# AO33/HiC_Genome_Assembler

Measured on AMD Instinct MI355X. Metric: Part1+Part2 wall-clock (s) and bins/s on N x N contact map, higher is better.
Workload: dtype f64

## Files before the change

hic_genome_assembler_amd/csrc/api.hip:

```cpp
#include <hip/hip_runtime.h>

#include <algorithm>
#include <cmath>
#include <cstdarg>
#include <climits>
#include <cstdio>
#include <cstdlib>
#include <cstring>
#include <numeric>
#include <string>
#include <type_traits>
#include <unordered_map>
#include <functional>
#include <chrono>
#include <vector>

#include "../../include/hicmi.h"
#include "hicmi_internal.h"
#include "devbuf.h"
#include "hyper.h"

using namespace hicmi;

static thread_local std::string g_err;
// ... 2792 lines not shown
        launch_p2_total_perm(c->dM2, c->ld2, c->d_pos2sel, (int)c->n_arr, c->d_T, c->d_scores, c->stream);
    }
    HIPCHK(hipGetLastError());
    HIPCHK(hipMemcpyAsync(c->pin_down, c->d_scores, sizeof(double), hipMemcpyDeviceToHost, c->stream));
    return HICMI_OK;
}
}

int hicmi_p2_arrangement_total(hicmi_ctx* c, double* total_out)
{
    if (!c || !total_out) return fail(HICMI_EINVAL, "bad arguments");
    int rc = arrangement_total_enqueue(c);
    if (rc) return rc;
    HIPCHK(sync_stream(c));
    memcpy(total_out, c->pin_down, sizeof(double));
    return HICMI_OK;
}

int hicmi_p2_arrangement_score(hicmi_ctx* c, double total, double* score_out)
{
    if (!c || !score_out) return fail(HICMI_EINVAL, "bad arguments");
    if (c->n_arr < 1) return fail(HICMI_EINVAL, "hicmi_p2_set_arrangement has not run");
    if (c->n_arr < 2) { *score_out = 0.0; return HICMI_OK; }
    HIPCHK(hipSetDevice(c->device));
    const int NB = kBaseSlabs;
    int rc = ensure(c->d_scores, NB);
    if (rc) return rc;
    {
        Timed t(c, F_P2_SCORE, 4.0 * (double)c->n_arr * (double)(c->n_arr - 1));
        launch_p2_base_partial(c->dM2, c->ld2, c->d_pos2sel, (int)c->n_arr, c->d_H, (int)c->n_arr, NB, c->d_scores, c->stream);
    }
    HIPCHK(hipGetLastError());
    double part[NB];
    rc = download(c, part, c->d_scores, sizeof(double) * NB);
    if (rc) return rc;
    double sum = 0.0;
    for (int b = 0; b < NB; b++) sum += part[b];
    *score_out = sum / total;
    return HICMI_OK;
}

int hicmi_p2_score_insertions(hicmi_ctx* c, int32_t new_id, double total, double* scores_out)
{
    if (!c || !scores_out) return fail(HICMI_EINVAL, "bad arguments");
    if (c->n_scaf < 1) return fail(HICMI_EINVAL, "hicmi_p2_layout has not run");
    if (new_id < 0 || new_id >= c->n_scaf) return fail(HICMI_EINVAL, "new scaffold out of range");
    const int64_t S = (int64_t)c->h_arr_id.size();
    if (c->n_arr < 1 || S < 1) return fail(HICMI_EINVAL, "hicmi_p2_set_arrangement has not run");
    for (int64_t j = 0; j < S; j++) if (c->h_arr_id[(size_t)j] == new_id) return fail(HICMI_EINVAL, "scaffold is already in the arrangement");
    const int new_len = c->h_scaf_len[(size_t)new_id];
    if (int rc = check_candidate_bins(c->n_arr + new_len)) return rc;
    HIPCHK(hipSetDevice(c->device));
    const int NB = kBaseSlabs;
    const int64_t n_out = NB + S + 2 * (S + 1);
    int rc = ensure(c->d_scores, n_out);
    if (rc) return rc;
    {
        const double nn = (double)c->n_arr;
        Timed t(c, F_P2_INSERT, 8.0 * (0.5 * nn * (nn - 1.0) + nn * nn + 2.0 * (double)(S + 1) * (double)new_len * nn));
        launch_p2_insert_delta(c->dM2, c->ld2, c->d_pos2sel, (int)c->n_arr, c->d_arr_packed + S, (int)S,
                               c->h_scaf_start[(size_t)new_id], new_len, c->d_H, NB, c->d_scores, c->stream);
    }
    HIPCHK(hipGetLastError());
    std::vector<double> host((size_t)n_out);
    rc = download(c, host.data(), c->d_scores, sizeof(double) * (size_t)n_out);
    if (rc) return rc;
    double base = 0.0;
    for (int b = 0; b < NB; b++) base += host[(size_t)b];
    double straddle = 0.0;
    for (int64_t g = 0; g <= S; g++) {
        if (g > 0) straddle += host[(size_t)(NB + g - 1)];
        for (int r = 0; r < 2; r++)
            scores_out[2 * g + r] = (base - straddle + host[(size_t)(NB + S + 2 * g + r)]) / total;
    }
    return HICMI_OK;
}

int hicmi_p2_window_tables(hicmi_ctx* c, int64_t k, const int8_t* orders, int64_t n_orders, const uint8_t* orients,
                           int64_t n_orients)
{
    if (!c || !orders || !orients || k < 1 || k > 8 || n_orders < 1 || n_orients < 1) return fail(HICMI_EINVAL, "bad arguments");
    for (int64_t i = 0; i < n_orders * k; i++) if (orders[i] < 0 || orders[i] >= k) return fail(HICMI_EINVAL, "order table entry out of range");
    HIPCHK(hipSetDevice(c->device));
    int rc = ensure(c->d_orders, n_orders * k);
    if (!rc) rc = ensure(c->d_orients, n_orients * k);
    if (rc) return rc;
    rc = upload(c, c->d_orders, orders, (size_t)(n_orders * k));
    if (rc) return rc;
    rc = upload(c, c->d_orients, orients, (size_t)(n_orients * k));
    if (rc) return rc;
    c->tab_k = (int)k; c->n_orders = n_orders; c->n_orients = n_orients;
    c->h_orders.assign(orders, orders + n_orders * k);
    c->h_orients.assign(orients, orients + n_orients * k);
    return HICMI_OK;
}

namespace {
int64_t window_c0(const hicmi_ctx* c, int64_t first, int64_t k)
{
    for (int64_t r = 0; r < c->n_orients; r++) {
        bool same = true;
        for (int64_t j = 0; j < k; j++) same = same && ((c->h_orients[(size_t)(r * k + j)] != 0) == (c->h_arr_rev[(size_t)(first + j)] != 0));
        if (same) return r;
    }
    return -1;
}

struct BatchCost { int64_t g_total = 0; int max_m = 0; double g_bytes = 0.0, d_bytes = 0.0, g_flops = 0.0; };

int fill_batch(hicmi_ctx* c, int64_t first0, int64_t count, int64_t k, std::vector<WindowBatchEntry>& wb, BatchCost& bc)
{
    const int64_t S = (int64_t)c->h_arr_id.size();
    if (c->n_arr < 1 || S < 1) return fail(HICMI_EINVAL, "hicmi_p2_set_arrangement has not run");
    if (k != c->tab_k) return fail(HICMI_EINVAL, "hicmi_p2_window_tables has not been called for k = %lld", (long long)k);
    if (first0 < 0 || count < 1 || first0 + count - 1 + k > S) return fail(HICMI_EINVAL, "window out of range");
    const int64_t n_cand = c->n_orders * c->n_orients;
    wb.assign((size_t)count, WindowBatchEntry{});
    int64_t g_total = 0; int max_m = 0; double g_bytes = 0.0, d_bytes = 0.0, g_flops = 0.0;
    for (int64_t wdx = 0; wdx < count; wdx++) {
        const int64_t first = first0 + wdx;
        WindowBatchEntry& e = wb[(size_t)wdx];
        memset(&e, 0, sizeof(e));
        const int p0 = c->h_arr_pos[(size_t)first], p1 = c->h_arr_pos[(size_t)(first + k)];
        e.p0 = p0; e.m = p1 - p0; e.g_off = g_total;
        for (int64_t j = 0; j < k; j++) {
            const int32_t sc = c->h_arr_id[(size_t)(first + j)];
// ... 451 lines not shown
    return HICMI_OK;
}


namespace {
void apply_insertion(int32_t* ids, uint8_t* rev, int64_t& S, int64_t gap, int32_t new_id, int32_t r)
{
    for (int64_t j = S; j > gap; j--) { ids[j] = ids[j - 1]; rev[j] = rev[j - 1]; }
    ids[gap] = new_id; rev[gap] = (uint8_t)(r ? 1 : 0);
    S++;
}

struct InsJob {
    hicmi_ctx* c; int32_t* ids; uint8_t* rev; int64_t S; const int32_t* new_ids; int64_t n_new;
    int64_t t = 0; double best = 0.0; bool device_ok = true;
};

int queue_insertions(hicmi_ctx* lead, const std::vector<InsJob*>& jobs)
{
    const int nj = (int)jobs.size();
    if (nj == 0) return HICMI_OK;
    const int NB = kBaseSlabs;
    static const int max_c = getenv("HICMI_P2_INS_MAXC") ? atoi(getenv("HICMI_P2_INS_MAXC")) : INS_MAXC;
    int64_t steps_max = 0;
    std::vector<size_t> blob_off((size_t)nj);
    size_t blob_bytes = 0;
    for (int j = 0; j < nj; j++) {
        InsJob& job = *jobs[(size_t)j];
        hicmi_ctx* c = job.c;
        int rc = hicmi_p2_set_arrangement(c, job.ids, job.rev, job.S);
        if (rc) return rc;
        if (c != lead) HIPCHK(sync_stream(c));
        const int64_t n_steps = job.n_new - job.t;
        int64_t n_max = c->n_arr;
        for (int64_t t = 0; t < n_steps; t++) n_max += c->h_scaf_len[(size_t)job.new_ids[job.t + t]];
        rc = check_candidate_bins(n_max);
        if (rc) return rc;
        const int64_t S_max = job.S + n_steps;
        rc = ensure(c->d_arr_packed2, 3 * std::max<int64_t>(S_max, c->n_scaf) + 2);
        if (!rc) rc = ensure(c->d_pos2sel2, c->n2);
        if (!rc) rc = ensure(c->d_ins_T, (1 + 2 * (int64_t)INS_MAXC) * n_max);
        if (!rc) rc = ensure(c->d_ins_partial, NB + n_max + 2 * (S_max + 1));
        if (rc) return rc;
        steps_max = std::max(steps_max, n_steps);
        blob_off[(size_t)j] = blob_bytes;
        blob_bytes += (sizeof(InsState) + sizeof(InsLog) * (size_t)n_steps + 15) & ~(size_t)15;
    }
    HIPCHK(hipSetDevice(lead->device));
    int rc = ensure(lead->d_ins_blob, (int64_t)blob_bytes);
    if (!rc) rc = ensure(lead->d_ins_steps, steps_max * nj);
    if (rc) return rc;
    std::vector<InsStep> table((size_t)(steps_max * nj));
    std::vector<int> max_n_used((size_t)steps_max, 0), max_S((size_t)steps_max, 0), max_n_arr((size_t)steps_max, 0);
    double algo = 0.0;
    for (int j = 0; j < nj; j++) {
        InsJob& job = *jobs[(size_t)j];
        hicmi_ctx* c = job.c;
        const int64_t n_steps = job.n_new - job.t;
        int64_t n_max = c->n_arr;
        for (int64_t t = 0; t < n_steps; t++) n_max += c->h_scaf_len[(size_t)job.new_ids[job.t + t]];
        InsState* st = reinterpret_cast<InsState*>(lead->d_ins_blob + blob_off[(size_t)j]);
        InsLog* log = reinterpret_cast<InsLog*>(lead->d_ins_blob + blob_off[(size_t)j] + sizeof(InsState));
        int32_t* packed[2] = {c->d_arr_packed, c->d_arr_packed2};
        int32_t* pos2sel[2] = {c->d_pos2sel, c->d_pos2sel2};
        int64_t n_arr = c->n_arr;
        for (int64_t t = 0; t < steps_max; t++) {
            InsStep& d = table[(size_t)(t * nj + j)];
            memset(&d, 0, sizeof(d));
            d.st = st;
            if (t >= n_steps) continue;
            const int cur = (int)(t & 1), nxt = cur ^ 1;
            const int32_t nid = job.new_ids[job.t + t];
            const int L = c->h_scaf_len[(size_t)nid];
            d.M2 = c->dM2; d.H = c->d_H; d.ld2 = c->ld2;
            d.pos_cur = pos2sel[cur]; d.pos_nxt = pos2sel[nxt]; d.packed_cur = packed[cur]; d.packed_nxt = packed[nxt];
            d.T_total = c->d_ins_T; d.T_cand = c->d_ins_T + n_max; d.work = c->d_ins_T + (1 + (int64_t)INS_MAXC) * n_max;
            d.partial = c->d_ins_partial; d.log = log + t;
            d.n_arr = (int32_t)n_arr; d.S = (int32_t)(job.S + t); d.L = L; d.new_start = c->h_scaf_start[(size_t)nid];
            d.new_id = nid; d.active = 1; d.step = (int32_t)t; d.last = t == n_steps - 1;
            max_n_used[(size_t)t] = std::max(max_n_used[(size_t)t], (int)(n_arr + L));
            max_S[(size_t)t] = std::max(max_S[(size_t)t], d.S);
            max_n_arr[(size_t)t] = std::max(max_n_arr[(size_t)t], (int)n_arr);
            const double nn = (double)n_arr, Ld = (double)L, sd = (double)d.S;
            algo += 8.0 * (0.5 * nn * (nn - 1.0) + nn * nn + 2.0 * (sd + 1.0) * Ld * nn) + 4.0 * (nn + Ld) * (nn + Ld);
            n_arr += L;
        }
    }
    rc = upload(lead, lead->d_ins_steps, table.data(), sizeof(InsStep) * table.size());
    if (rc) return rc;
    {
        Timed timed(lead, F_P2_INSERT, algo);
        launch_insb_reset(lead->d_ins_steps, nj, lead->stream);
        for (int64_t t = 0; t < steps_max; t++) {
            const InsStep* st_t = lead->d_ins_steps + t * nj;
            const int nu = max_n_used[(size_t)t];
            launch_insb_fast(st_t, nj, max_S[(size_t)t], max_n_arr[(size_t)t], NB, lead->stream);
            launch_insb_shortlist(st_t, nj, max_S[(size_t)t], max_n_arr[(size_t)t], NB, kNearTop, max_c, lead->stream);
            launch_insb_diag_cand(st_t, nj, nu, lead->stream);
            launch_insb_cost(st_t, nj, nu, lead->stream);
            launch_insb_apply(st_t, nj, nu, lead->stream);
        }
    }
    HIPCHK(hipGetLastError());
    std::vector<unsigned char> blob(blob_bytes);
    rc = download(lead, blob.data(), lead->d_ins_blob, blob_bytes);
    if (rc) return rc;
    if (getenv("HICMI_PART2_PROFILE")) {
        int64_t hist[5] = {0, 0, 0, 0, 0}, all_direct = 0;
        for (int64_t t = 0; t < steps_max; t++) {
            int mx = -1, ran = 0;
            for (int j = 0; j < nj; j++) {
                if (t >= jobs[(size_t)j]->n_new - jobs[(size_t)j]->t) continue;
                const InsState* hs = reinterpret_cast<const InsState*>(blob.data() + blob_off[(size_t)j]);
                if (hs->fail >= 0 && t >= hs->fail) continue;
                const InsLog* hl = reinterpret_cast<const InsLog*>(blob.data() + blob_off[(size_t)j] + sizeof(InsState));
                const int ns = hl[t].n_short;
                hist[ns < 0 ? 0 : (ns > 3 ? 4 : ns + 1)]++;
                mx = std::max(mx, ns);
                ran++;
            }
            if (ran && mx < 0) all_direct++;
        }
        fprintf(stderr, "[hicmi] insertion short lists: direct %lld, literal with 0:%lld 1:%lld 2:%lld 3+:%lld candidates; "
                        "lock steps without any literal pass: %lld of %lld\n",
                (long long)hist[0], (long long)hist[1], (long long)hist[2], (long long)hist[3], (long long)hist[4],
                (long long)all_direct, (long long)steps_max);
    }
    for (int j = 0; j < nj; j++) {
        InsJob& job = *jobs[(size_t)j];
        const int64_t n_steps = job.n_new - job.t;
        const InsState* hst = reinterpret_cast<const InsState*>(blob.data() + blob_off[(size_t)j]);
        const InsLog* hlog = reinterpret_cast<const InsLog*>(blob.data() + blob_off[(size_t)j] + sizeof(InsState));
        const int64_t done = hst->fail >= 0 ? std::min<int64_t>(hst->fail, n_steps) : n_steps;
        for (int64_t t = 0; t < done; t++) {
            if (hlog[t].gap < 0 || hlog[t].gap > job.S) return fail(HICMI_ESTATE, "insertion log out of range");
            apply_insertion(job.ids, job.rev, job.S, hlog[t].gap, job.new_ids[job.t + t], hlog[t].rev);
            job.best = hlog[t].best;
        }
        job.t += done;
        hicmi_ctx* c = job.c;
        c->n_arr = 0; c->h_arr_id.clear(); c->h_arr_rev.clear(); c->h_arr_pos.clear(); c->h_pos2sel.clear();
    }
    return HICMI_OK;
}

int check_insert_job(const InsJob& job, int64_t S0)
{
    hicmi_ctx* c = job.c;
    if (!c || !job.ids || !job.rev || !job.new_ids || S0 < 1 || job.n_new < 1) return fail(HICMI_EINVAL, "bad arguments");
// ... 1278 lines not shown
```

hic_genome_assembler_amd/csrc/hicmi_internal.h:

```cpp
#pragma once
#include <hip/hip_runtime.h>
#include <stdint.h>

#include <atomic>
#include <functional>

#include "liftmap.h"
#include "span.h"
#include "ends.h"
#include "anchor.h"
#include "pairs.h"
#include "seats.h"
#include "links.h"
#include "split.h"

namespace hicmi {

inline void ensure_dynamic_lds(const void* func, std::atomic<int>& have, size_t bytes)
{
    if ((int)bytes > have.load(std::memory_order_relaxed)) {
        (void)hipFuncSetAttribute(func, hipFuncAttributeMaxDynamicSharedMemorySize, (int)bytes);
        have.store((int)bytes, std::memory_order_relaxed);
    }
}
// ... 159 lines not shown
    }
}
#endif

int  sort_padded_size(int n);
int  sort_workgroups(int n);
size_t sort_scratch_bytes(int n);
struct SortExtras {
    const int32_t* row_list = nullptr; int n_list = 0;
    uint8_t* tie_flag = nullptr; unsigned* tie_count = nullptr; unsigned tie_limit = 0;
    uint16_t* tie_bits = nullptr; int64_t ld_bits = 0;
    int max_workgroups = 0;
    int avoid_xcc = -1; unsigned* row_counter = nullptr;
};
static constexpr int GETREG_XCC_ID = 20 | (0 << 6) | (3 << 11);
int nnchain_local_xcc(const NNChainOptions& o, int n);
void launch_sort_rows(const double* C, int64_t ldc, const int32_t* order, const int32_t* inv, const double* np_sum,
                      const double* seq_sum, int n, void* scratch, uint16_t* R, int64_t ldr, int row_first, int row_stride,
                      hipStream_t s, const SortExtras& x = SortExtras());
void launch_rank_rows_tied(const uint16_t* R_storage, const uint16_t* tie_bits, int64_t ld_bits, const int32_t* order,
                           const int32_t* inv, int n, const int32_t* row_list, int n_list, uint16_t* rank, int64_t ldr,
                           hipStream_t s, int32_t* done = nullptr);
void launch_rank_relabel(const uint16_t* rank_storage, uint16_t* rank, int64_t ldr, int n, const int32_t* order, int row_first,
                         int row_stride, hipStream_t s);
size_t sort_radix_scratch_bytes(int n);
void launch_rank_rows_radix(const double* C, int64_t ldc, const int32_t* order, const int32_t* inv, const double* np_sum,
                            const double* seq_sum, int n, void* scratch, uint16_t* rank, int64_t ldr, int row_first,
                            int row_stride, hipStream_t s);
void launch_rank_invert(const uint16_t* R, uint16_t* rank, int64_t ldr, int n, int row_first, int row_stride, hipStream_t s,
                        const int32_t* row_list = nullptr, int n_list = 0);
void launch_similarity_row(const double* C, int64_t ldc, const int32_t* order, const double* np_sum,
                           const double* seq_sum, int n, int row, double* out, hipStream_t s);

void launch_p2_select(const double* C, int64_t ldc, const int32_t* sel, int n, double* M2, int64_t ld2, hipStream_t s);
void launch_p2_total(const double* M2, int64_t ld2, int n, double* T, double* total, hipStream_t s);
void launch_p2_score_exact(const double* M2, int64_t ld2, const int32_t* perms, int n_cand, int n_used, double total,
                           double* T, double* work, double* scores, hipStream_t s);
void launch_p2_score(const double* M2, int64_t ld2, const int32_t* perms, int n_cand, int n_used, const double* H,
                     double inv_total_unused, double total, double* scores, hipStream_t s);

void launch_p2_total_perm(const double* M2, int64_t ld2, const int32_t* d_perm, int n, double* T, double* total,
                          hipStream_t s);

struct WindowDesc {
    int32_t start[8];
    int32_t len[8];
    int32_t off[8];
    uint8_t rev[8];
};
void launch_arr_materialize(const int32_t* packed, int S, const int32_t* scaf_start, const int32_t* scaf_len, int n_arr,
                            int32_t* pos2sel, hipStream_t s);
void launch_p2_base_partial(const double* M2, int64_t ld2, const int32_t* pos2sel, int n_arr, const double* H, int n_tot,
                            int n_blocks, double* out, hipStream_t s);
void launch_p2_insert_delta(const double* M2, int64_t ld2, const int32_t* pos2sel, int n_arr, const int32_t* arr_pos,
                            int S, int new_start, int L, const double* H, int n_base_blocks, double* out, hipStream_t s);
struct WindowBatchEntry {
    WindowDesc w;
    int32_t p0, m;
    int64_t g_off;
    int32_t c0, pad;
};
void launch_p2_window_batch_G(const double* M2, int64_t ld2, const int32_t* pos2sel, int n, const WindowBatchEntry* wb, int n_win,
                              int max_m, const double* H, double* G_all, hipStream_t s);
void launch_p2_window_batch_delta(const double* M2, int64_t ld2, const int32_t* pos2sel, int n, int k,
                                  const WindowBatchEntry* wb, int n_win, int max_m, const int8_t* orders, const uint8_t* orients,
                                  int n_ord, int n_ori, const double* H, const double* G_all, double* delta_all, hipStream_t s);


int64_t window_table_doubles(int k);
void launch_p2_window_tables(const double* M2, int64_t ld2, const int32_t* pos2sel, int n, int k,
                             const WindowBatchEntry* wb, const WindowBatchEntry* h_wb, int n_win, int max_m, const double* H,
                             double* tables, hipStream_t s);
void launch_p2_window_candidates(int k, int n_win, const int8_t* orders, const uint8_t* orients, int n_ord, int n_ori,
                                 const double* tables, double* delta_all, hipStream_t s);
struct NearEntry { int32_t cand, pad; double fast; };
int window_near_blocks(int n_ord);
void launch_p2_window_near(const double* M2, int64_t ld2, const int32_t* pos2sel, int n, int k,
                           const WindowBatchEntry* wb, const WindowBatchEntry* h_wb, int n_win, int max_m, const int8_t* orders,
                           const uint8_t* orients, int n_ord, int n_ori, const double* H, double* tables, int whole, double total,
                           double cur_fast, double floor, double near_top, double* part, int32_t* count, NearEntry* near, int cap,
                           hipStream_t s);

__device__ __forceinline__ double wave_sum_s(double v)
{
#pragma unroll
    for (int off = 32; off >= 1; off >>= 1) v += __shfl_xor(v, off, 64);
    return v;
}

__device__ __forceinline__ double block_sum_256(double v, double* s_w)
{
    v = wave_sum_s(v);
    if ((threadIdx.x & 63) == 0) s_w[threadIdx.x >> 6] = v;
    __syncthreads();
    return (s_w[0] + s_w[1]) + (s_w[2] + s_w[3]);
}

__device__ __forceinline__ void base_partial_body(const double* __restrict__ M2, int64_t ld2, const int32_t* p, int n_arr,
                                                  const double* __restrict__ H, int n_tot, int blk, int n_blk,
                                                  double* __restrict__ out)
{
    __shared__ double s_w[4];
    const int lane = threadIdx.x & 63, wave = threadIdx.x >> 6;
    const double hn = H[n_tot - 1];
    double acc = 0.0;
    for (int a = blk * 4 + wave; a < n_arr - 1; a += n_blk * 4) {
        const double* __restrict__ row = M2 + (int64_t)p[a] * ld2;
#pragma unroll 4
// ... 12 lines not shown
    double mx = -__builtin_inf();
    int at = 0x7fffffff;
    for (int i = tid; i < n_cand; i += 256) {
        const double v = scores[i];
        if (counts(i) && isfinite(v) && v > mx) { mx = v; at = i; }
    }
    s_val[tid] = mx; s_idx[tid] = at;
    if (tid == 0) s_cnt = 0;
    __syncthreads();
    for (int w = 128; w >= 1; w >>= 1) {
        if (tid < w) {
            const double o = s_val[tid + w];
            const int oi = s_idx[tid + w];
            if (o > s_val[tid] || (o == s_val[tid] && oi < s_idx[tid])) { s_val[tid] = o; s_idx[tid] = oi; }
        }
        __syncthreads();
    }
    const double top = s_val[0];
    const int first = s_idx[0];
    if (first == 0x7fffffff) {
        if (tid == 0) { best[0] = -1; best[1] = 0; }
        return;
    }
    const double thr = top - fabs(top) * near_top;
    int near = 0;
    for (int i = tid; i < n_cand; i += 256) {
        const double v = scores[i];
        near += counts(i) && isfinite(v) && v >= thr;
    }
    if (near) atomicAdd(&s_cnt, near);
    __syncthreads();
    if (tid == 0) { best[0] = first; best[1] = s_cnt; }
}

static constexpr int INS_MAXC = 8;
struct InsState {
    int32_t fail;
    int32_t n_short;
    int32_t direct, pad;
    int32_t gap[INS_MAXC], rev[INS_MAXC], idx[INS_MAXC];
    double total;
    double lit[INS_MAXC];
};
struct InsLog { int32_t gap, rev; double best; int32_t n_short, pad; };
struct InsStep {
    const double* M2; const double* H; int64_t ld2;
    const int32_t* pos_cur; int32_t* pos_nxt;
    const int32_t* packed_cur; int32_t* packed_nxt;
    double *T_total, *T_cand, *work, *partial;
    InsState* st; InsLog* log;
    int32_t n_arr, S, L, new_start, new_id, active, step, last;
};
void launch_insb_reset(const InsStep* steps, int n_chrom, hipStream_t s);
void launch_insb_fast(const InsStep* steps, int n_chrom, int max_S, int max_n_arr, int n_base_blocks, hipStream_t s);
void launch_insb_shortlist(const InsStep* steps, int n_chrom, int max_S, int max_n_arr, int n_base_blocks, double near_top,
                           int max_c, hipStream_t s);
void launch_insb_diag_cand(const InsStep* steps, int n_chrom, int max_n_used, hipStream_t s);
void launch_insb_cost(const InsStep* steps, int n_chrom, int max_n_used, hipStream_t s);
void launch_insb_apply(const InsStep* steps, int n_chrom, int max_n_used, hipStream_t s);

static constexpr int SUP_BASE_SLABS = 64;
static constexpr int SUP_MAX_S = 4096;
struct SupRec {
    const double* M2; const double* H; int64_t ld2;
    const int32_t* pos;
    const int32_t* arr_pos;
    double* partial;
    double* scores;
    int32_t* best;
    double total;
    int32_t n, S, j, start, L, cur_rev;
};
void launch_sup(const SupRec* recs, int n_rec, int max_S, int max_n, double near_top, hipStream_t s);

static constexpr int BRK_BASE_SLABS = 64;
struct BrkRec {
    const double* M2; const double* H; int64_t ld2;
    const int32_t* pos;
    double* X;
    double* pq;
    double* base;
    double* scores;
    int32_t* best;
    double total;
    int64_t wg0;
    int32_t n, B, L, min_piece;
    int32_t n_base, pad;
};
void launch_brk(const BrkRec* recs, int n_rec, int64_t n_wg, double near_top, hipStream_t s);

static constexpr int INV_BASE_SLABS = 64;
static constexpr int INV_MAX_S = 4096;
static constexpr double INV_MAX_WORK = 1e13;
struct InvRec {
    const double* M2; const double* H; int64_t ld2;
    const int32_t* pos;
    const int32_t* arr_pos;
    double* base;
    double* scores;
    int32_t* best;
    double total;
    int64_t wg0;
    int32_t n, S, i, n_j;
    int32_t max_span, n_base;
};
void launch_inv(const InvRec* recs, int n_rec, int64_t n_wg, double near_top, hipStream_t s);

// ... 181 lines not shown
```

hic_genome_assembler_amd/csrc/k_part2_search.hip:

```cpp
#include "hicmi_internal.h"

namespace hicmi {

__device__ __forceinline__ double block_sum_1024(double v, double* s_w)
{
    v = wave_sum_s(v);
    if ((threadIdx.x & 63) == 0) s_w[threadIdx.x >> 6] = v;
    __syncthreads();
    double acc = 0.0;
#pragma unroll
    for (int i = 0; i < 16; i++) acc += s_w[i];
    return acc;
}

static size_t perm_lds_bytes(int n) { return (((size_t)n * sizeof(int32_t)) + 15) & ~(size_t)15; }

__global__ __launch_bounds__(256) void k_arr_materialize(const int32_t* __restrict__ packed, int S,
                                                         const int32_t* __restrict__ scaf_start,
                                                         const int32_t* __restrict__ scaf_len, int n_arr,
                                                         int32_t* __restrict__ pos2sel)
{
    const int32_t* __restrict__ arr_id = packed;
    const int32_t* __restrict__ arr_pos = packed + S;
    const int32_t* __restrict__ arr_rev = packed + 2 * S + 1;
    int q = blockIdx.x * 256 + threadIdx.x;
    if (q >= n_arr) return;
    int lo = 0, hi = S;
    while (hi - lo > 1) {
        int mid = (lo + hi) >> 1;
        if (arr_pos[mid] <= q) lo = mid; else hi = mid;
    }
    int sc = arr_id[lo], off = q - arr_pos[lo], len = scaf_len[sc];
    pos2sel[q] = scaf_start[sc] + (arr_rev[lo] ? len - 1 - off : off);
}

void launch_arr_materialize(const int32_t* packed, int S, const int32_t* scaf_start, const int32_t* scaf_len, int n_arr,
                            int32_t* pos2sel, hipStream_t s)
{
    if (n_arr <= 0) return;
    hipLaunchKernelGGL(k_arr_materialize, dim3((n_arr + 255) / 256), dim3(256), 0, s, packed, S, scaf_start, scaf_len,
                       n_arr, pos2sel);
}

__global__ __launch_bounds__(256) void k_p2_base_partial(const double* __restrict__ M2, int64_t ld2,
                                                         const int32_t* __restrict__ pos2sel, int n_arr,
                                                         const double* __restrict__ H, int n_tot,
                                                         double* __restrict__ partial)
{
    extern __shared__ __attribute__((aligned(16))) unsigned char smem[];
    int32_t* p = reinterpret_cast<int32_t*>(smem);
    for (int q = threadIdx.x; q < n_arr; q += 256) p[q] = pos2sel[q];
    __syncthreads();
    base_partial_body(M2, ld2, p, n_arr, H, n_tot, blockIdx.x, gridDim.x, partial + blockIdx.x);
}

static std::atomic<int> g_lds_base{0}, g_lds_straddle{0}, g_lds_cross{0}, g_lds_wdelta{0}, g_lds_wdelta1{0}, g_lds_wdelta_blk{0}, g_lds_wG{0}, g_lds_insb_base{0}, g_lds_insb_fast{0};

void launch_p2_base_partial(const double* M2, int64_t ld2, const int32_t* pos2sel, int n_arr, const double* H, int n_tot,
                            int n_blocks, double* out, hipStream_t s)
{
    ensure_dynamic_lds(reinterpret_cast<const void*>(k_p2_base_partial), g_lds_base, perm_lds_bytes(n_arr));
    hipLaunchKernelGGL(k_p2_base_partial, dim3(n_blocks), dim3(256), perm_lds_bytes(n_arr), s, M2, ld2, pos2sel, n_arr, H,
                       n_tot, out);
}

__device__ __forceinline__ void straddle_body(const double* __restrict__ M2, int64_t ld2, const int32_t* p, int n_arr,
                                              const int32_t* __restrict__ arr_pos, int g, int L,
                                              const double* __restrict__ H, double* s_w, double* __restrict__ out)
{
    const int lane = threadIdx.x & 63, wave = threadIdx.x >> 6;
    const int P0 = arr_pos[g], P1 = arr_pos[g + 1];
    const int len = P1 - P0, n_out = n_arr - len;
    double acc = 0.0;
    for (int u = P0 + wave; u < P1; u += 16) {
        const double* __restrict__ row = M2 + (int64_t)p[u] * ld2;
#pragma unroll 8
        for (int qq = lane; qq < n_out; qq += 64) {
            const bool before = qq < P0;
            const int pos = before ? qq : qq + len;
            const int d = before ? u - pos : pos - u;
            const double w = H[d + L - 1] - H[d - 1];
            const double v = row[p[pos]] * w;
            acc += before ? -v : v;
        }
    }
    double sum = block_sum_1024(acc, s_w);
    if (threadIdx.x == 0) out[0] = sum;
}

__device__ __forceinline__ void cross_body(const double* __restrict__ M2, int64_t ld2, const int32_t* p, int n_arr,
                                           const int32_t* __restrict__ arr_pos, int g, int r, int new_start, int L,
                                           const double* __restrict__ H, double* s_w, double* __restrict__ out)
{
    const int lane = threadIdx.x & 63, wave = threadIdx.x >> 6;
    const int P = arr_pos[g];
    const double hn = H[n_arr + L - 1];
    double acc = 0.0;
    for (int e = wave; e < L; e += 16) {
        const int xe = new_start + (r ? L - 1 - e : e);
        const double* __restrict__ row = M2 + (int64_t)xe * ld2;
#pragma unroll 4
        for (int q = lane; q < n_arr; q += 64) {
            int d = q < P ? (P + e - q) : (q + L - (P + e));
            acc += row[p[q]] * (hn - H[d - 1]);
        }
        for (int e2 = e + 1 + lane; e2 < L; e2 += 64) {
            int x2 = new_start + (r ? L - 1 - e2 : e2);
            acc += row[x2] * (hn - H[e2 - e - 1]);
        }
    }
    double sum = block_sum_1024(acc, s_w);
    if (threadIdx.x == 0) out[0] = sum;
}

__global__ __launch_bounds__(1024) void k_p2_insert_straddle(const double* __restrict__ M2, int64_t ld2,
                                                            const int32_t* __restrict__ pos2sel, int n_arr,
                                                            const int32_t* __restrict__ arr_pos, int L,
                                                            const double* __restrict__ H, double* __restrict__ D)
{
    extern __shared__ __attribute__((aligned(16))) unsigned char smem[];
    int32_t* p = reinterpret_cast<int32_t*>(smem);
    __shared__ double s_w[16];
    for (int q = threadIdx.x; q < n_arr; q += 1024) p[q] = pos2sel[q];
    __syncthreads();
    straddle_body(M2, ld2, p, n_arr, arr_pos, blockIdx.x, L, H, s_w, D + blockIdx.x);
}

__global__ __launch_bounds__(1024) void k_p2_insert_cross(const double* __restrict__ M2, int64_t ld2,
                                                         const int32_t* __restrict__ pos2sel, int n_arr,
                                                         const int32_t* __restrict__ arr_pos, int new_start, int L,
                                                         const double* __restrict__ H, double* __restrict__ cross)
{
    extern __shared__ __attribute__((aligned(16))) unsigned char smem[];
    int32_t* p = reinterpret_cast<int32_t*>(smem);
    __shared__ double s_w[16];
    for (int q = threadIdx.x; q < n_arr; q += 1024) p[q] = pos2sel[q];
    __syncthreads();
    cross_body(M2, ld2, p, n_arr, arr_pos, blockIdx.x >> 1, blockIdx.x & 1, new_start, L, H, s_w, cross + blockIdx.x);
}

void launch_p2_insert_delta(const double* M2, int64_t ld2, const int32_t* pos2sel, int n_arr, const int32_t* arr_pos,
                            int S, int new_start, int L, const double* H, int n_base_blocks, double* out, hipStream_t s)
{
    const size_t lds = perm_lds_bytes(n_arr);
    launch_p2_base_partial(M2, ld2, pos2sel, n_arr, H, n_arr + L, n_base_blocks, out, s);
    ensure_dynamic_lds(reinterpret_cast<const void*>(k_p2_insert_straddle), g_lds_straddle, lds);
    ensure_dynamic_lds(reinterpret_cast<const void*>(k_p2_insert_cross), g_lds_cross, lds);
    hipLaunchKernelGGL(k_p2_insert_straddle, dim3(S), dim3(1024), lds, s, M2, ld2, pos2sel, n_arr, arr_pos, L, H,
                       out + n_base_blocks);
    hipLaunchKernelGGL(k_p2_insert_cross, dim3(2 * (S + 1)), dim3(1024), lds, s, M2, ld2, pos2sel, n_arr, arr_pos, new_start,
                       L, H, out + n_base_blocks + S);
}

__global__ __launch_bounds__(256) void k_insb_base(const InsStep* __restrict__ steps, int n_base_blocks)
{
    extern __shared__ __attribute__((aligned(16))) unsigned char smem[];
    int32_t* p = reinterpret_cast<int32_t*>(smem);
    const InsStep& d = steps[blockIdx.y];
    if (!d.active || d.st->fail >= 0) return;
    for (int q = threadIdx.x; q < d.n_arr; q += 256) p[q] = d.pos_cur[q];
    __syncthreads();
    base_partial_body(d.M2, d.ld2, p, d.n_arr, d.H, d.n_arr + d.L, blockIdx.x, n_base_blocks, d.partial + blockIdx.x);
}

__global__ __launch_bounds__(256) void k_insb_fast(const InsStep* __restrict__ steps, int n_base_blocks, int n_row_blocks,
                                                   int n_cross_blocks)
{
    extern __shared__ __attribute__((aligned(16))) unsigned char smem[];
    __shared__ double s_w[4];
    const InsStep& d = steps[blockIdx.y];
    if (!d.active || d.st->fail >= 0) return;
    const int S = d.S, n_arr = d.n_arr, L = d.L;
    const int lane = threadIdx.x & 63, wave = threadIdx.x >> 6;
    const int32_t* __restrict__ p = d.pos_cur;
    const int32_t* __restrict__ arr_pos = d.packed_cur + S;
    const double* __restrict__ H = d.H;
    const int n_base_here = (int)gridDim.x - n_row_blocks - n_cross_blocks;
    const int bx = (int)blockIdx.x - n_base_here;
    if (bx < 0) {
        const int slab = blockIdx.x;
        int32_t* pl = reinterpret_cast<int32_t*>(smem);
        for (int q = threadIdx.x; q < n_arr; q += 256) pl[q] = p[q];
        __syncthreads();
        base_partial_body(d.M2, d.ld2, pl, n_arr, H, n_arr + L, slab, n_base_blocks, d.partial + slab);
        return;
    }
    if (bx < n_row_blocks) {
        const int u = bx * 4 + wave;
        if (u >= n_arr) return;
        int below = 0;
        for (int j = lane; j <= S; j += 64) below += arr_pos[j] <= u;
#pragma unroll
        for (int off = 32; off >= 1; off >>= 1) below += __shfl_xor(below, off, 64);
        const int g = below - 1;
        const int P0 = arr_pos[g], P1 = arr_pos[g + 1];
        const double* __restrict__ row = d.M2 + (int64_t)p[u] * d.ld2;
        double acc = 0.0;
#pragma unroll 4
        for (int pos = lane; pos < P0; pos += 64) {
            const int dd = u - pos;
            acc -= row[p[pos]] * (H[dd + L - 1] - H[dd - 1]);
        }
#pragma unroll 4
        for (int pos = P1 + lane; pos < n_arr; pos += 64) {
            const int dd = pos - u;
            acc += row[p[pos]] * (H[dd + L - 1] - H[dd - 1]);
        }
        acc = wave_sum_s(acc);
        if (lane == 0) d.partial[n_base_blocks + u] = acc;
        return;
    }
    const int c = bx - n_row_blocks;
    if (c >= 2 * (S + 1)) return;
    const int g = c >> 1, r = c & 1, P = arr_pos[g];
    const double hn = H[n_arr + L - 1];
    double acc = 0.0;
    for (int e = wave; e < L; e += 4) {
        const int xe = d.new_start + (r ? L - 1 - e : e);
        const double* __restrict__ row = d.M2 + (int64_t)xe * d.ld2;
#pragma unroll 4
        for (int q = lane; q < n_arr; q += 64) {
            const int dd = q < P ? (P + e - q) : (q + L - (P + e));
            acc += row[p[q]] * (hn - H[dd - 1]);
        }
        for (int e2 = e + 1 + lane; e2 < L; e2 += 64) {
            const int x2 = d.new_start + (r ? L - 1 - e2 : e2);
            acc += row[x2] * (hn - H[e2 - e - 1]);
        }
    }
    const double sum = block_sum_256(acc, s_w);
    if (threadIdx.x == 0) d.partial[n_base_blocks + n_arr + c] = sum;
}

void launch_insb_fast(const InsStep* steps, int n_chrom, int max_S, int max_n_arr, int n_base_blocks, hipStream_t s)
{
    const size_t lds = perm_lds_bytes(max_n_arr);
    const int n_row_blocks = (max_n_arr + 3) / 4, n_cross_blocks = 2 * (max_S + 1);
    static const bool split = getenv("HICMI_P2_INSB_SPLIT") != nullptr;
    if (split) {
        ensure_dynamic_lds(reinterpret_cast<const void*>(k_insb_base), g_lds_insb_base, lds);
        hipLaunchKernelGGL(k_insb_base, dim3(n_base_blocks, n_chrom), dim3(256), lds, s, steps, n_base_blocks);
    }
    ensure_dynamic_lds(reinterpret_cast<const void*>(k_insb_fast), g_lds_insb_fast, lds);
    hipLaunchKernelGGL(k_insb_fast, dim3(n_row_blocks + n_cross_blocks + (split ? 0 : n_base_blocks), n_chrom), dim3(256), lds, s,
                       steps, n_base_blocks, n_row_blocks, n_cross_blocks);
}

static constexpr int G_TILE = 2048;
static constexpr int G_TMAX = 8;

template <bool H_IN_LDS>
__global__ __launch_bounds__(256) void k_p2_window_G(const double* __restrict__ M2, int64_t ld2,
                                                     const int32_t* __restrict__ pos2sel, int n,
                                                     const WindowBatchEntry* __restrict__ wb,
                                                     const double* H, double* __restrict__ G_all)
{
    extern __shared__ __attribute__((aligned(16))) unsigned char smem_g[];
    __shared__ double vals[G_TILE];
    __shared__ double part[4][64];
    const WindowBatchEntry& we = wb[blockIdx.y];
    const int p0 = we.p0, m = we.m;
    const int x = blockIdx.x, tid = threadIdx.x, tl = tid & 63, seg = tid >> 6;
    if (x >= m) return;
    double* __restrict__ G = G_all + we.g_off;
    const double* __restrict__ row = M2 + (int64_t)pos2sel[p0 + x] * ld2;
    const double hn = H[n - 1];
    if (H_IN_LDS) {
        double* hl = reinterpret_cast<double*>(smem_g);
        for (int i = tid; i < n; i += 256) hl[i] = H[i];
        __syncthreads();
        H = hl;
    }
    const int n_out = n - m;
    for (int tbase = 0; tbase < m; tbase += 64 * G_TMAX) {
        double acc[G_TMAX];
#pragma unroll
        for (int i = 0; i < G_TMAX; i++) acc[i] = 0.0;
        for (int base = 0; base < n_out; base += G_TILE) {
            const int cnt = n_out - base < G_TILE ? n_out - base : G_TILE;
            __syncthreads();
            for (int e = tid; e < cnt; e += 256) {
                int qq = base + e;
                vals[e] = row[pos2sel[qq < p0 ? qq : qq + m]];
            }
            __syncthreads();
            const int e0 = (cnt * seg) >> 2, e1 = (cnt * (seg + 1)) >> 2;
#pragma unroll
            for (int i = 0; i < G_TMAX; i++) {
                const int t = tbase + i * 64 + tl;
                if (t < m) {
                    const int pt = p0 + t;
                    double a = acc[i];
                    for (int e = e0; e < e1; e++) {
                        int qq = base + e;
                        int d = qq < p0 ? pt - qq : qq + m - pt;
                        a += vals[e] * (hn - H[d - 1]);
                    }
                    acc[i] = a;
// ... 134 lines not shown
```

Measured before the change: 125,600.

## Restructure insertion-scoring kernels with LDS staging, gap batching and fused row/base passes

Rewrites the insertion scoring kernel so base-partial and per-row straddle work share one pass over each row. The permutation, H table and arrangement positions are staged in LDS when the problem fits under a size cap. The cross kernel now evaluates eight gap positions per block, reusing each loaded matrix row across those gaps, and loads are batched to raise memory-level parallelism. The single-insertion API is switched to this batched path and the old straddle/cross kernels are removed. This adds register pressure from the per-gap accumulators and larger LDS use, and moves per-gap straddle summation onto the host.

```diff
diff --git a/hic_genome_assembler_amd/csrc/api.hip b/hic_genome_assembler_amd/csrc/api.hip
--- a/hic_genome_assembler_amd/csrc/api.hip
+++ b/hic_genome_assembler_amd/csrc/api.hip
@@ -2868,14 +2868,28 @@
     if (int rc = check_candidate_bins(c->n_arr + new_len)) return rc;
     HIPCHK(hipSetDevice(c->device));
     const int NB = kBaseSlabs;
-    const int64_t n_out = NB + S + 2 * (S + 1);
+    const int64_t n_arr = c->n_arr;
+    const int64_t n_out = NB + n_arr + 2 * (S + 1);
     int rc = ensure(c->d_scores, n_out);
+    if (!rc) rc = ensure(c->d_ins_blob, (int64_t)sizeof(InsState));
+    if (!rc) rc = ensure(c->d_ins_steps, 1);
+    if (rc) return rc;
+    InsStep d;
+    memset(&d, 0, sizeof(d));
+    d.M2 = c->dM2; d.H = c->d_H; d.ld2 = c->ld2;
+    d.pos_cur = c->d_pos2sel; d.packed_cur = c->d_arr_packed; d.partial = c->d_scores;
+    d.st = reinterpret_cast<InsState*>(c->d_ins_blob.get());
+    d.n_arr = (int32_t)n_arr; d.S = (int32_t)S; d.L = new_len; d.new_start = c->h_scaf_start[(size_t)new_id];
+    d.new_id = new_id; d.active = 1; d.last = 1;
+    rc = upload(c, c->d_ins_steps, &d, sizeof(d));
     if (rc) return rc;
     {
         const double nn = (double)c->n_arr;
+        const bool staged = n_arr + new_len <= INSB_STAGE_MAX;
         Timed t(c, F_P2_INSERT, 8.0 * (0.5 * nn * (nn - 1.0) + nn * nn + 2.0 * (double)(S + 1) * (double)new_len * nn));
-        launch_p2_insert_delta(c->dM2, c->ld2, c->d_pos2sel, (int)c->n_arr, c->d_arr_packed + S, (int)S,
-                               c->h_scaf_start[(size_t)new_id], new_len, c->d_H, NB, c->d_scores, c->stream);
+        launch_insb_reset(c->d_ins_steps, 1, c->stream);
+        launch_insb_fast(c->d_ins_steps, 1, (int)S, NB, staged ? (int)(n_arr + new_len) : 0, staged ? 0 : (int)n_arr,
+                         c->stream);
     }
     HIPCHK(hipGetLastError());
     std::vector<double> host((size_t)n_out);
@@ -2885,9 +2899,13 @@
     for (int b = 0; b < NB; b++) base += host[(size_t)b];
     double straddle = 0.0;
     for (int64_t g = 0; g <= S; g++) {
-        if (g > 0) straddle += host[(size_t)(NB + g - 1)];
+        if (g > 0) {
+            double inc = 0.0;
+            for (int u = c->h_arr_pos[(size_t)(g - 1)]; u < c->h_arr_pos[(size_t)g]; u++) inc += host[(size_t)(NB + u)];
+            straddle += inc;
+        }
         for (int r = 0; r < 2; r++)
-            scores_out[2 * g + r] = (base - straddle + host[(size_t)(NB + S + 2 * g + r)]) / total;
+            scores_out[2 * g + r] = (base - straddle + host[(size_t)(NB + n_arr + 2 * g + r)]) / total;
     }
     return HICMI_OK;
 }
@@ -3445,6 +3463,7 @@
     if (rc) return rc;
     std::vector<InsStep> table((size_t)(steps_max * nj));
     std::vector<int> max_n_used((size_t)steps_max, 0), max_S((size_t)steps_max, 0), max_n_arr((size_t)steps_max, 0);
+    std::vector<int> stage_n((size_t)steps_max, 0), over_n_arr((size_t)steps_max, 0);
     double algo = 0.0;
     for (int j = 0; j < nj; j++) {
         InsJob& job = *jobs[(size_t)j];
@@ -3474,6 +3493,8 @@
             max_n_used[(size_t)t] = std::max(max_n_used[(size_t)t], (int)(n_arr + L));
             max_S[(size_t)t] = std::max(max_S[(size_t)t], d.S);
             max_n_arr[(size_t)t] = std::max(max_n_arr[(size_t)t], (int)n_arr);
+            if (n_arr + L <= INSB_STAGE_MAX) stage_n[(size_t)t] = std::max(stage_n[(size_t)t], (int)(n_arr + L));
+            else over_n_arr[(size_t)t] = std::max(over_n_arr[(size_t)t], (int)n_arr);
             const double nn = (double)n_arr, Ld = (double)L, sd = (double)d.S;
             algo += 8.0 * (0.5 * nn * (nn - 1.0) + nn * nn + 2.0 * (sd + 1.0) * Ld * nn) + 4.0 * (nn + Ld) * (nn + Ld);
             n_arr += L;
@@ -3487,7 +3508,7 @@
         for (int64_t t = 0; t < steps_max; t++) {
             const InsStep* st_t = lead->d_ins_steps + t * nj;
             const int nu = max_n_used[(size_t)t];
-            launch_insb_fast(st_t, nj, max_S[(size_t)t], max_n_arr[(size_t)t], NB, lead->stream);
+            launch_insb_fast(st_t, nj, max_S[(size_t)t], NB, stage_n[(size_t)t], over_n_arr[(size_t)t], lead->stream);
             launch_insb_shortlist(st_t, nj, max_S[(size_t)t], max_n_arr[(size_t)t], NB, kNearTop, max_c, lead->stream);
             launch_insb_diag_cand(st_t, nj, nu, lead->stream);
             launch_insb_cost(st_t, nj, nu, lead->stream);
diff --git a/hic_genome_assembler_amd/csrc/hicmi_internal.h b/hic_genome_assembler_amd/csrc/hicmi_internal.h
--- a/hic_genome_assembler_amd/csrc/hicmi_internal.h
+++ b/hic_genome_assembler_amd/csrc/hicmi_internal.h
@@ -235,8 +235,6 @@
                             int32_t* pos2sel, hipStream_t s);
 void launch_p2_base_partial(const double* M2, int64_t ld2, const int32_t* pos2sel, int n_arr, const double* H, int n_tot,
                             int n_blocks, double* out, hipStream_t s);
-void launch_p2_insert_delta(const double* M2, int64_t ld2, const int32_t* pos2sel, int n_arr, const int32_t* arr_pos,
-                            int S, int new_start, int L, const double* H, int n_base_blocks, double* out, hipStream_t s);
 struct WindowBatchEntry {
     WindowDesc w;
     int32_t p0, m;
@@ -355,7 +353,9 @@
     int32_t n_arr, S, L, new_start, new_id, active, step, last;
 };
 void launch_insb_reset(const InsStep* steps, int n_chrom, hipStream_t s);
-void launch_insb_fast(const InsStep* steps, int n_chrom, int max_S, int max_n_arr, int n_base_blocks, hipStream_t s);
+static constexpr int INSB_STAGE_MAX = 2400;
+static constexpr int INSB_G = 8;
+void launch_insb_fast(const InsStep* steps, int n_chrom, int max_S, int n_base_blocks, int stage_n, int over_n_arr, hipStream_t s);
 void launch_insb_shortlist(const InsStep* steps, int n_chrom, int max_S, int max_n_arr, int n_base_blocks, double near_top,
                            int max_c, hipStream_t s);
 void launch_insb_diag_cand(const InsStep* steps, int n_chrom, int max_n_used, hipStream_t s);
diff --git a/hic_genome_assembler_amd/csrc/k_part2_search.hip b/hic_genome_assembler_amd/csrc/k_part2_search.hip
--- a/hic_genome_assembler_amd/csrc/k_part2_search.hip
+++ b/hic_genome_assembler_amd/csrc/k_part2_search.hip
@@ -1,17 +1,6 @@
 #include "hicmi_internal.h"
 
 namespace hicmi {
-
-__device__ __forceinline__ double block_sum_1024(double v, double* s_w)
-{
-    v = wave_sum_s(v);
-    if ((threadIdx.x & 63) == 0) s_w[threadIdx.x >> 6] = v;
-    __syncthreads();
-    double acc = 0.0;
-#pragma unroll
-    for (int i = 0; i < 16; i++) acc += s_w[i];
-    return acc;
-}
 
 static size_t perm_lds_bytes(int n) { return (((size_t)n * sizeof(int32_t)) + 15) & ~(size_t)15; }
 
@@ -54,7 +43,7 @@
     base_partial_body(M2, ld2, p, n_arr, H, n_tot, blockIdx.x, gridDim.x, partial + blockIdx.x);
 }
 
-static std::atomic<int> g_lds_base{0}, g_lds_straddle{0}, g_lds_cross{0}, g_lds_wdelta{0}, g_lds_wdelta1{0}, g_lds_wdelta_blk{0}, g_lds_wG{0}, g_lds_insb_base{0}, g_lds_insb_fast{0};
+static std::atomic<int> g_lds_base{0}, g_lds_wdelta{0}, g_lds_wdelta1{0}, g_lds_wdelta_blk{0}, g_lds_wG{0}, g_lds_insb_base{0}, g_lds_insb_fast{0};
 
 void launch_p2_base_partial(const double* M2, int64_t ld2, const int32_t* pos2sel, int n_arr, const double* H, int n_tot,
                             int n_blocks, double* out, hipStream_t s)
@@ -64,186 +53,198 @@
                        n_tot, out);
 }
 
-__device__ __forceinline__ void straddle_body(const double* __restrict__ M2, int64_t ld2, const int32_t* p, int n_arr,
-                                              const int32_t* __restrict__ arr_pos, int g, int L,
-                                              const double* __restrict__ H, double* s_w, double* __restrict__ out)
+
+static constexpr int INSB_BATCH = 8, INSB_CROSS_BATCH = 4;
+
+template <typename T> using gptr = const __attribute__((address_space(1))) T*;
+template <typename T> __device__ __forceinline__ gptr<T> as_global(const T* p) { return (gptr<T>)p; }
+
+static size_t insb_lds_bytes(int stage_n, int max_S, int over_n_arr)
+{
+    const size_t staged = stage_n > 0 ? (size_t)stage_n * 12 + (size_t)(max_S + 1) * 4 + 16 : 0;
+    const size_t over = over_n_arr > 0 ? perm_lds_bytes(over_n_arr) : 0;
+    return staged > over ? staged : over;
+}
+
+template <bool ROW, bool BASE, typename PI, typename PA, typename PD>
+__device__ __forceinline__ void insb_rows(const InsStep& d, PI p, PA ap, PD Ht, int blk, int n_base_blocks, double* s_w)
 {
     const int lane = threadIdx.x & 63, wave = threadIdx.x >> 6;
-    const int P0 = arr_pos[g], P1 = arr_pos[g + 1];
-    const int len = P1 - P0, n_out = n_arr - len;
-    double acc = 0.0;
-    for (int u = P0 + wave; u < P1; u += 16) {
-        const double* __restrict__ row = M2 + (int64_t)p[u] * ld2;
-#pragma unroll 8
-        for (int qq = lane; qq < n_out; qq += 64) {
-            const bool before = qq < P0;
-            const int pos = before ? qq : qq + len;
-            const int d = before ? u - pos : pos - u;
-            const double w = H[d + L - 1] - H[d - 1];
-            const double v = row[p[pos]] * w;
-            acc += before ? -v : v;
-        }
-    }
-    double sum = block_sum_1024(acc, s_w);
-    if (threadIdx.x == 0) out[0] = sum;
-}
-
-__device__ __forceinline__ void cross_body(const double* __restrict__ M2, int64_t ld2, const int32_t* p, int n_arr,
-                                           const int32_t* __restrict__ arr_pos, int g, int r, int new_start, int L,
-                                           const double* __restrict__ H, double* s_w, double* __restrict__ out)
-{
-    const int lane = threadIdx.x & 63, wave = threadIdx.x >> 6;
-    const int P = arr_pos[g];
-    const double hn = H[n_arr + L - 1];
-    double acc = 0.0;
-    for (int e = wave; e < L; e += 16) {
-        const int xe = new_start + (r ? L - 1 - e : e);
-        const double* __restrict__ row = M2 + (int64_t)xe * ld2;
-#pragma unroll 4
-        for (int q = lane; q < n_arr; q += 64) {
-            int d = q < P ? (P + e - q) : (q + L - (P + e));
-            acc += row[p[q]] * (hn - H[d - 1]);
-        }
-        for (int e2 = e + 1 + lane; e2 < L; e2 += 64) {
-            int x2 = new_start + (r ? L - 1 - e2 : e2);
-            acc += row[x2] * (hn - H[e2 - e - 1]);
-        }
-    }
-    double sum = block_sum_1024(acc, s_w);
-    if (threadIdx.x == 0) out[0] = sum;
-}
-
-__global__ __launch_bounds__(1024) void k_p2_insert_straddle(const double* __restrict__ M2, int64_t ld2,
-                                                            const int32_t* __restrict__ pos2sel, int n_arr,
-                                                            const int32_t* __restrict__ arr_pos, int L,
-                                                            const double* __restrict__ H, double* __restrict__ D)
-{
-    extern __shared__ __attribute__((aligned(16))) unsigned char smem[];
-    int32_t* p = reinterpret_cast<int32_t*>(smem);
-    __shared__ double s_w[16];
-    for (int q = threadIdx.x; q < n_arr; q += 1024) p[q] = pos2sel[q];
-    __syncthreads();
-    straddle_body(M2, ld2, p, n_arr, arr_pos, blockIdx.x, L, H, s_w, D + blockIdx.x);
-}
-
-__global__ __launch_bounds__(1024) void k_p2_insert_cross(const double* __restrict__ M2, int64_t ld2,
-                                                         const int32_t* __restrict__ pos2sel, int n_arr,
-                                                         const int32_t* __restrict__ arr_pos, int new_start, int L,
-                                                         const double* __restrict__ H, double* __restrict__ cross)
-{
-    extern __shared__ __attribute__((aligned(16))) unsigned char smem[];
-    int32_t* p = reinterpret_cast<int32_t*>(smem);
-    __shared__ double s_w[16];
-    for (int q = threadIdx.x; q < n_arr; q += 1024) p[q] = pos2sel[q];
-    __syncthreads();
-    cross_body(M2, ld2, p, n_arr, arr_pos, blockIdx.x >> 1, blockIdx.x & 1, new_start, L, H, s_w, cross + blockIdx.x);
-}
-
-void launch_p2_insert_delta(const double* M2, int64_t ld2, const int32_t* pos2sel, int n_arr, const int32_t* arr_pos,
-                            int S, int new_start, int L, const double* H, int n_base_blocks, double* out, hipStream_t s)
-{
-    const size_t lds = perm_lds_bytes(n_arr);
-    launch_p2_base_partial(M2, ld2, pos2sel, n_arr, H, n_arr + L, n_base_blocks, out, s);
-    ensure_dynamic_lds(reinterpret_cast<const void*>(k_p2_insert_straddle), g_lds_straddle, lds);
-    ensure_dynamic_lds(reinterpret_cast<const void*>(k_p2_insert_cross), g_lds_cross, lds);
-    hipLaunchKernelGGL(k_p2_insert_straddle, dim3(S), dim3(1024), lds, s, M2, ld2, pos2sel, n_arr, arr_pos, L, H,
-                       out + n_base_blocks);
-    hipLaunchKernelGGL(k_p2_insert_cross, dim3(2 * (S + 1)), dim3(1024), lds, s, M2, ld2, pos2sel, n_arr, arr_pos, new_start,
-                       L, H, out + n_base_blocks + S);
-}
-
-__global__ __launch_bounds__(256) void k_insb_base(const InsStep* __restrict__ steps, int n_base_blocks)
-{
-    extern __shared__ __attribute__((aligned(16))) unsigned char smem[];
-    int32_t* p = reinterpret_cast<int32_t*>(smem);
-    const InsStep& d = steps[blockIdx.y];
-    if (!d.active || d.st->fail >= 0) return;
-    for (int q = threadIdx.x; q < d.n_arr; q += 256) p[q] = d.pos_cur[q];
-    __syncthreads();
-    base_partial_body(d.M2, d.ld2, p, d.n_arr, d.H, d.n_arr + d.L, blockIdx.x, n_base_blocks, d.partial + blockIdx.x);
-}
-
-__global__ __launch_bounds__(256) void k_insb_fast(const InsStep* __restrict__ steps, int n_base_blocks, int n_row_blocks,
-                                                   int n_cross_blocks)
+    const int S = d.S, n_arr = d.n_arr, L = d.L;
+    const double hn = as_global(d.H)[n_arr + L - 1];
+    double base = 0.0;
+    for (int a = blk * 4 + wave; a < n_arr; a += n_base_blocks * 4) {
+        const gptr<double> row = as_global(d.M2) + (int64_t)p[a] * d.ld2;
+        if (ROW) {
+            int below = 0;
+            for (int j = lane; j <= S; j += 64) below += ap[j] <= a;
+#pragma unroll
+            for (int off = 32; off >= 1; off >>= 1) below += __shfl_xor(below, off, 64);
+            const int g = below - 1;
+            const int P0 = ap[g], P1 = ap[g + 1];
+            double acc = 0.0;
+            for (int c0 = lane; c0 - lane < P0; c0 += 64 * INSB_BATCH) {
+                double v[INSB_BATCH];
+#pragma unroll
+                for (int k = 0; k < INSB_BATCH; k++) { const int pos = c0 + 64 * k; v[k] = pos < P0 ? row[p[pos]] : 0.0; }
+#pragma unroll
+                for (int k = 0; k < INSB_BATCH; k++) {
+                    const int pos = c0 + 64 * k, dd = a - pos;
+                    if (pos < P0) acc -= v[k] * (Ht[dd + L - 1] - Ht[dd - 1]);
+                }
+            }
+            for (int c0 = P1 + lane; c0 - lane < n_arr; c0 += 64 * INSB_BATCH) {
+                double v[INSB_BATCH];
+#pragma unroll
+                for (int k = 0; k < INSB_BATCH; k++) { const int pos = c0 + 64 * k; v[k] = pos < n_arr ? row[p[pos]] : 0.0; }
+#pragma unroll
+                for (int k = 0; k < INSB_BATCH; k++) {
+                    const int pos = c0 + 64 * k, dd = pos - a;
+                    if (pos < n_arr) acc += v[k] * (Ht[dd + L - 1] - Ht[dd - 1]);
+                }
+            }
+            acc = wave_sum_s(acc);
+            if (lane == 0) d.partial[n_base_blocks + a] = acc;
+        }
+        if (BASE) {
+            for (int b0 = a + 1 + lane; b0 - lane < n_arr; b0 += 64 * INSB_BATCH) {
+                double v[INSB_BATCH];
+#pragma unroll
+                for (int k = 0; k < INSB_BATCH; k++) { const int b = b0 + 64 * k; v[k] = b < n_arr ? row[p[b]] : 0.0; }
+#pragma unroll
+                for (int k = 0; k < INSB_BATCH; k++) { const int b = b0 + 64 * k; if (b < n_arr) base += v[k] * (hn - Ht[b - a - 1]); }
+            }
+        }
+    }
+    if (BASE) {
+        const double sum = block_sum_256(base, s_w);
+        if (threadIdx.x == 0) d.partial[blk] = sum;
+    }
+}
+
+template <bool ROW, bool BASE>
+__device__ __forceinline__ void insb_rows_role(const InsStep& d, int blk, int n_base_blocks, unsigned char* smem, int stage_n,
+                                               int max_S, int over_n_arr, double* s_w)
+{
+    const int S = d.S, n_arr = d.n_arr, L = d.L;
+    if (n_arr + L <= stage_n && S <= max_S) {
+        double* Hl = reinterpret_cast<double*>(smem);
+        int32_t* pl = reinterpret_cast<int32_t*>(smem + (size_t)stage_n * 8);
+        int32_t* apl = pl + stage_n;
+        for (int q = threadIdx.x; q < n_arr; q += 256) pl[q] = as_global(d.pos_cur)[q];
+        for (int i = threadIdx.x; i < n_arr + L - 1; i += 256) Hl[i] = as_global(d.H)[i];
+        if (ROW) for (int j = threadIdx.x; j <= S; j += 256) apl[j] = as_global(d.packed_cur)[S + j];
+        __syncthreads();
+        insb_rows<ROW, BASE>(d, (const int32_t*)pl, (const int32_t*)apl, (const double*)Hl, blk, n_base_blocks, s_w);
+        return;
+    }
+    if (n_arr <= over_n_arr) {
+        int32_t* pl = reinterpret_cast<int32_t*>(smem);
+        for (int q = threadIdx.x; q < n_arr; q += 256) pl[q] = as_global(d.pos_cur)[q];
+        __syncthreads();
+        insb_rows<ROW, BASE>(d, (const int32_t*)pl, as_global(d.packed_cur) + S, as_global(d.H), blk, n_base_blocks, s_w);
+        return;
+    }
+    insb_rows<ROW, BASE>(d, as_global(d.pos_cur), as_global(d.packed_cur) + S, as_global(d.H), blk, n_base_blocks, s_w);
+}
+
+__global__ __launch_bounds__(256) void k_insb_base(const InsStep* __restrict__ steps, int n_base_blocks, int stage_n, int max_S,
+                                                   int over_n_arr)
 {
     extern __shared__ __attribute__((aligned(16))) unsigned char smem[];
     __shared__ double s_w[4];
     const InsStep& d = steps[blockIdx.y];
     if (!d.active || d.st->fail >= 0) return;
+    insb_rows_role<false, true>(d, blockIdx.x, n_base_blocks, smem, stage_n, max_S, over_n_arr, s_w);
+}
+
+template <typename PI, typename PD>
+__device__ __forceinline__ void insb_cross(const InsStep& d, PI p, PD Ht, int g0, int r, int n_base_blocks, double (*s_w)[4])
+{
+    const int lane = threadIdx.x & 63, wave = threadIdx.x >> 6;
     const int S = d.S, n_arr = d.n_arr, L = d.L;
-    const int lane = threadIdx.x & 63, wave = threadIdx.x >> 6;
-    const int32_t* __restrict__ p = d.pos_cur;
-    const int32_t* __restrict__ arr_pos = d.packed_cur + S;
-    const double* __restrict__ H = d.H;
-    const int n_base_here = (int)gridDim.x - n_row_blocks - n_cross_blocks;
-    const int bx = (int)blockIdx.x - n_base_here;
-    if (bx < 0) {
-        const int slab = blockIdx.x;
-        int32_t* pl = reinterpret_cast<int32_t*>(smem);
-        for (int q = threadIdx.x; q < n_arr; q += 256) pl[q] = p[q];
-        __syncthreads();
-        base_partial_body(d.M2, d.ld2, pl, n_arr, H, n_arr + L, slab, n_base_blocks, d.partial + slab);
-        return;
-    }
-    if (bx < n_row_blocks) {
-        const int u = bx * 4 + wave;
-        if (u >= n_arr) return;
-        int below = 0;
-        for (int j = lane; j <= S; j += 64) below += arr_pos[j] <= u;
-#pragma unroll
-        for (int off = 32; off >= 1; off >>= 1) below += __shfl_xor(below, off, 64);
-        const int g = below - 1;
-        const int P0 = arr_pos[g], P1 = arr_pos[g + 1];
-        const double* __restrict__ row = d.M2 + (int64_t)p[u] * d.ld2;
-        double acc = 0.0;
-#pragma unroll 4
-        for (int pos = lane; pos < P0; pos += 64) {
-            const int dd = u - pos;
-            acc -= row[p[pos]] * (H[dd + L - 1] - H[dd - 1]);
-        }
-#pragma unroll 4
-        for (int pos = P1 + lane; pos < n_arr; pos += 64) {
-            const int dd = pos - u;
-            acc += row[p[pos]] * (H[dd + L - 1] - H[dd - 1]);
-        }
-        acc = wave_sum_s(acc);
-        if (lane == 0) d.partial[n_base_blocks + u] = acc;
-        return;
-    }
-    const int c = bx - n_row_blocks;
-    if (c >= 2 * (S + 1)) return;
-    const int g = c >> 1, r = c & 1, P = arr_pos[g];
-    const double hn = H[n_arr + L - 1];
-    double acc = 0.0;
+    const gptr<int32_t> arr_pos = as_global(d.packed_cur) + S;
+    const double hn = as_global(d.H)[n_arr + L - 1];
+    int P[INSB_G];
+    double acc[INSB_G];
+#pragma unroll
+    for (int g = 0; g < INSB_G; g++) { P[g] = arr_pos[g0 + g <= S ? g0 + g : S]; acc[g] = 0.0; }
     for (int e = wave; e < L; e += 4) {
         const int xe = d.new_start + (r ? L - 1 - e : e);
-        const double* __restrict__ row = d.M2 + (int64_t)xe * d.ld2;
-#pragma unroll 4
-        for (int q = lane; q < n_arr; q += 64) {
-            const int dd = q < P ? (P + e - q) : (q + L - (P + e));
-            acc += row[p[q]] * (hn - H[dd - 1]);
+        const gptr<double> row = as_global(d.M2) + (int64_t)xe * d.ld2;
+        for (int q0 = lane; q0 - lane < n_arr; q0 += 64 * INSB_CROSS_BATCH) {
+            double v[INSB_CROSS_BATCH];
+#pragma unroll
+            for (int k = 0; k < INSB_CROSS_BATCH; k++) { const int q = q0 + 64 * k; v[k] = q < n_arr ? row[p[q]] : 0.0; }
+#pragma unroll
+            for (int k = 0; k < INSB_CROSS_BATCH; k++) {
+                const int q = q0 + 64 * k;
+                if (q < n_arr) {
+#pragma unroll
+                    for (int g = 0; g < INSB_G; g++) {
+                        const int dd = q < P[g] ? (P[g] + e - q) : (q + L - (P[g] + e));
+                        acc[g] += v[k] * (hn - Ht[dd - 1]);
+                    }
+                }
+            }
         }
         for (int e2 = e + 1 + lane; e2 < L; e2 += 64) {
             const int x2 = d.new_start + (r ? L - 1 - e2 : e2);
-            acc += row[x2] * (hn - H[e2 - e - 1]);
-        }
-    }
-    const double sum = block_sum_256(acc, s_w);
-    if (threadIdx.x == 0) d.partial[n_base_blocks + n_arr + c] = sum;
-}
-
-void launch_insb_fast(const InsStep* steps, int n_chrom, int max_S, int max_n_arr, int n_base_blocks, hipStream_t s)
-{
-    const size_t lds = perm_lds_bytes(max_n_arr);
-    const int n_row_blocks = (max_n_arr + 3) / 4, n_cross_blocks = 2 * (max_S + 1);
+            const double t = row[x2] * (hn - Ht[e2 - e - 1]);
+#pragma unroll
+            for (int g = 0; g < INSB_G; g++) acc[g] += t;
+        }
+    }
+#pragma unroll
+    for (int g = 0; g < INSB_G; g++) {
+        const double sum = block_sum_256(acc[g], s_w[g]);
+        if (threadIdx.x == 0 && g0 + g <= S) d.partial[n_base_blocks + n_arr + 2 * (g0 + g) + r] = sum;
+    }
+}
+
+__global__ __launch_bounds__(256) void k_insb_fast(const InsStep* __restrict__ steps, int n_base_blocks, int n_cross_blocks,
+                                                   int with_base, int stage_n, int max_S, int over_n_arr)
+{
+    extern __shared__ __attribute__((aligned(16))) unsigned char smem[];
+    __shared__ double s_w[INSB_G][4];
+    const InsStep& d = steps[blockIdx.y];
+    if (!d.active || d.st->fail >= 0) return;
+    const int S = d.S, n_arr = d.n_arr, L = d.L;
+    if ((int)blockIdx.x < n_base_blocks) {
+        if ((int)blockIdx.x * 4 >= n_arr && !with_base) return;
+        if (with_base) insb_rows_role<true, true>(d, blockIdx.x, n_base_blocks, smem, stage_n, max_S, over_n_arr, s_w[0]);
+        else insb_rows_role<true, false>(d, blockIdx.x, n_base_blocks, smem, stage_n, max_S, over_n_arr, s_w[0]);
+        return;
+    }
+    const int c = (int)blockIdx.x - n_base_blocks;
+    const int g0 = (c >> 1) * INSB_G, r = c & 1;
+    if (g0 > S) return;
+    if (n_arr + L > stage_n) {
+        insb_cross(d, as_global(d.pos_cur), as_global(d.H), g0, r, n_base_blocks, s_w);
+        return;
+    }
+    double* tbl = reinterpret_cast<double*>(smem);
+    int32_t* pl = reinterpret_cast<int32_t*>(smem + (size_t)stage_n * 8);
+    for (int q = threadIdx.x; q < n_arr; q += 256) pl[q] = as_global(d.pos_cur)[q];
+    for (int i = threadIdx.x; i < n_arr + L - 1; i += 256) tbl[i] = as_global(d.H)[i];
+    __syncthreads();
+    insb_cross(d, (const int32_t*)pl, (const double*)tbl, g0, r, n_base_blocks, s_w);
+}
+
+void launch_insb_fast(const InsStep* steps, int n_chrom, int max_S, int n_base_blocks, int stage_n, int over_n_arr, hipStream_t s)
+{
+    if (stage_n > INSB_STAGE_MAX) stage_n = 0;
+    const size_t lds = insb_lds_bytes(stage_n, max_S, over_n_arr);
+    const int n_cross_blocks = 2 * ((max_S + INSB_G) / INSB_G);
     static const bool split = getenv("HICMI_P2_INSB_SPLIT") != nullptr;
     if (split) {
         ensure_dynamic_lds(reinterpret_cast<const void*>(k_insb_base), g_lds_insb_base, lds);
-        hipLaunchKernelGGL(k_insb_base, dim3(n_base_blocks, n_chrom), dim3(256), lds, s, steps, n_base_blocks);
+        hipLaunchKernelGGL(k_insb_base, dim3(n_base_blocks, n_chrom), dim3(256), lds, s, steps, n_base_blocks, stage_n, max_S,
+                           over_n_arr);
     }
     ensure_dynamic_lds(reinterpret_cast<const void*>(k_insb_fast), g_lds_insb_fast, lds);
-    hipLaunchKernelGGL(k_insb_fast, dim3(n_row_blocks + n_cross_blocks + (split ? 0 : n_base_blocks), n_chrom), dim3(256), lds, s,
-                       steps, n_base_blocks, n_row_blocks, n_cross_blocks);
+    hipLaunchKernelGGL(k_insb_fast, dim3(n_base_blocks + n_cross_blocks, n_chrom), dim3(256), lds, s, steps, n_base_blocks,
+                       n_cross_blocks, split ? 0 : 1, stage_n, max_S, over_n_arr);
 }
 
 static constexpr int G_TILE = 2048;
```

After: 122,500. -2.5%, worse.
